# dphoyes/OpenCL-Structure-from-Motion

Hardware: NVIDIA B200
Metric: matched frame-pairs/sec at 1241x376 (higher is better)
Workload: dtype u8

## Files before the change

opencl-structure-from-motion_b200/csrc/outliers.cu:

```cuda
#include "visocu_internal.cuh"
#include "outliers.cuh"
#include <cstdio>
#include <cstdlib>
#include <cstring>
#include <mutex>
#include <type_traits>
#include <utility>
#include <vector>

namespace {

constexpr int NIL = 0xFFFF;
constexpr uint16_t DEAD = 0xFFFF;

__host__ __device__ inline int ro_edge_capacity(int n) { return (int)(3.04f * (float)n) + 64; }
__host__ __device__ inline size_t ro_smem_bytes(int n) {
  return (((size_t)12 * ro_edge_capacity(n) + 15) & ~(size_t)15) + (size_t)4 * n + 16;
}

struct Mesh {
  uint16_t* __restrict__ nx; uint16_t* __restrict__ pv; uint16_t* __restrict__ og;
  const uint32_t* __restrict__ pt;
  int* bump; int ecap; volatile int* fail;
  int guard;

  __device__ __forceinline__ int org(int e) const { return og[e]; }
  __device__ __forceinline__ int dest(int e) const { return og[e ^ 1]; }
  __device__ __forceinline__ int onext(int e) const { return nx[e]; }
  __device__ __forceinline__ int oprev(int e) const { return pv[e]; }
  __device__ __forceinline__ int lnext(int e) const { return pv[e ^ 1]; }
  __device__ __forceinline__ int rprev(int e) const { return nx[e ^ 1]; }
  __device__ __forceinline__ int px(int v) const { return (int)(pt[v] & 0xFFFFu); }
  __device__ __forceinline__ int py(int v) const { return (int)(pt[v] >> 16); }
  __device__ __forceinline__ bool tick() { return --guard >= 0; }
  __device__ __forceinline__ int ccw(int a, int b, int c) const { return ccw_pts(pt[a], pt[b], pt[c]); }
  __device__ __forceinline__ long long incircle(int a, int b, int c, int d) const { return incircle_pts(pt[a], pt[b], pt[c], pt[d]); }
  static __device__ __forceinline__ int ccw_pts(uint32_t A, uint32_t B, uint32_t C) {
    const int cx = (int)(C & 0xFFFF), cy = (int)(C >> 16);
    const int ax = (int)(A & 0xFFFF) - cx, ay = (int)(A >> 16) - cy;
    const int bx = (int)(B & 0xFFFF) - cx, by = (int)(B >> 16) - cy;
    return ax * by - ay * bx;
  }
  static __device__ __forceinline__ long long incircle_pts(uint32_t A, uint32_t B, uint32_t C, uint32_t D) {
    const int dx = (int)(D & 0xFFFF), dy = (int)(D >> 16);
    const int adx = (int)(A & 0xFFFF) - dx, ady = (int)(A >> 16) - dy;
    const int bdx = (int)(B & 0xFFFF) - dx, bdy = (int)(B >> 16) - dy;
    const int cdx = (int)(C & 0xFFFF) - dx, cdy = (int)(C >> 16) - dy;
    const int al = adx * adx + ady * ady, bl = bdx * bdx + bdy * bdy, cl = cdx * cdx + cdy * cdy;
    return (long long)al * (bdx * cdy - cdx * bdy) + (long long)bl * (cdx * ady - adx * cdy) + (long long)cl * (adx * bdy - bdx * ady);
  }
};

struct FreeList { int head, tail; };

template <bool W>
__device__ __forceinline__ int make_edge(Mesh& m, FreeList& fl, int a, int b) {
  int e;
  if (fl.head != NIL) {
    e = fl.head;
    fl.head = (e == fl.tail) ? NIL : m.nx[e];
  } else {
    int k = 0;
    if (!W || (threadIdx.x & 31) == 0) k = atomicAdd(m.bump, 1);
    if (W) k = __shfl_sync(0xFFFFFFFFu, k, 0);
    if (k >= m.ecap) { *m.fail = 1; e = 0; } else e = 2 * k;
  }
  m.nx[e] = (uint16_t)e; m.pv[e] = (uint16_t)e; m.og[e] = (uint16_t)a;
  m.nx[e + 1] = (uint16_t)(e + 1); m.pv[e + 1] = (uint16_t)(e + 1); m.og[e + 1] = (uint16_t)b;
  return e;
}
__device__ __forceinline__ void insert_after(Mesh& m, int x, int e) {
  const int n = m.nx[x];
  m.nx[e] = (uint16_t)n; m.pv[e] = (uint16_t)x;
  m.pv[n] = (uint16_t)e; m.nx[x] = (uint16_t)e;
}
__device__ __forceinline__ void unlink(Mesh& m, int e) {
  const int n = m.nx[e], p = m.pv[e];
  m.nx[p] = (uint16_t)n; m.pv[n] = (uint16_t)p;
}
template <bool W>
__device__ __forceinline__ int connect(Mesh& m, FreeList& fl, int a, int b) {
  const int e = make_edge<W>(m, fl, m.dest(a), m.org(b));
  insert_after(m, m.lnext(a), e);
  insert_after(m, b, e ^ 1);
  return e;
}
__device__ __forceinline__ void remove_edge(Mesh& m, FreeList& fl, int e) {
  unlink(m, e); unlink(m, e ^ 1);
  e &= ~1;
  m.og[e] = DEAD; m.og[e + 1] = DEAD;
  if (fl.head == NIL) { fl.head = fl.tail = e; } else { m.nx[e] = (uint16_t)fl.head; fl.head = e; }
}

struct Handles { int ldo, rdo; };

template <bool W>
__device__ Handles merge(Mesh& m, FreeList& fl, Handles L, Handles R, int axis) {
  int ldo = L.ldo, ldi = L.rdo, rdi = R.ldo, rdo = R.rdo;
  if (axis == 1) {
    while (m.py(m.dest(ldo)) < m.py(m.org(ldo)) && m.tick()) ldo = m.rprev(ldo);
    while (m.py(m.dest(m.onext(ldi))) > m.py(m.org(ldi)) && m.tick()) ldi = m.onext(ldi) ^ 1;
    while (m.py(m.dest(rdi)) < m.py(m.org(rdi)) && m.tick()) rdi = m.rprev(rdi);
    while (m.py(m.dest(m.onext(rdo))) > m.py(m.org(rdo)) && m.tick()) rdo = m.onext(rdo) ^ 1;
  }
  bool changed;
  do {
    changed = false;
    if (m.ccw(m.org(ldi), m.dest(ldi), m.org(rdi)) > 0) { ldi = m.lnext(ldi); changed = true; }
    if (m.ccw(m.dest(rdi), m.org(rdi), m.org(ldi)) > 0) { rdi = m.rprev(rdi); changed = true; }
  } while (changed && m.tick());
  int basel = connect<W>(m, fl, rdi ^ 1, ldi);
  if (m.org(ldi) == m.org(ldo)) ldo = basel ^ 1;
  if (m.org(rdi) == m.org(rdo)) rdo = basel;
  while (m.tick()) {
    const int lowerright = m.org(basel), lowerleft = m.dest(basel);
    int lcand = m.onext(basel ^ 1), rcand = m.oprev(basel);
    int upperleft = m.dest(lcand), upperright = m.dest(rcand);
    const int lnx0 = m.onext(lcand), rnx0 = m.oprev(rcand);
    const int lapex0 = m.dest(lnx0), rapex0 = m.dest(rnx0);
    bool leftfinished, rightfinished, ldel0, rdel0, right_first = false;
    if (W) {
      const int lane = threadIdx.x & 31;
      int myv = rapex0;
      myv = lane == 4 ? lapex0 : myv; myv = lane == 3 ? upperright : myv; myv = lane == 2 ? upperleft : myv;
      myv = lane == 1 ? lowerright : myv; myv = lane == 0 ? lowerleft : myv;
      const uint32_t myp = m.pt[myv];
      const int sh = 4 * min(lane, 7);
#define RO_PICK(table) __shfl_sync(0xFFFFFFFFu, myp, (int)(((table) >> sh) & 7u))
      const uint32_t P = RO_PICK(0x01032u), Q = RO_PICK(0x05200u), R = RO_PICK(0x03411u);
      const uint32_t A = RO_PICK(0x20000u), B = RO_PICK(0x01100u), C = RO_PICK(0x13200u), D = RO_PICK(0x35400u);
#undef RO_PICK
      const unsigned cpos = __ballot_sync(0xFFFFFFFFu, Mesh::ccw_pts(P, Q, R) > 0);
      const unsigned ipos = __ballot_sync(0xFFFFFFFFu, Mesh::incircle_pts(A, B, C, D) > 0);
      leftfinished = !(cpos & 1u); rightfinished = !(cpos & 2u);
      ldel0 = !leftfinished && lnx0 != (basel ^ 1) && (cpos & 4u) && (ipos & 4u);
      rdel0 = !rightfinished && rnx0 != basel && (cpos & 8u) && (ipos & 8u);
      right_first = (ipos & 16u) != 0;
    } else {
      leftfinished = m.ccw(upperleft, lowerleft, lowerright) <= 0;
      rightfinished = m.ccw(upperright, lowerleft, lowerright) <= 0;
      ldel0 = !leftfinished && lnx0 != (basel ^ 1) && m.ccw(lowerleft, upperleft, lapex0) > 0 &&
              m.incircle(lowerleft, lowerright, upperleft, lapex0) > 0;
      rdel0 = !rightfinished && rnx0 != basel && m.ccw(lowerright, rapex0, upperright) > 0 &&
              m.incircle(lowerleft, lowerright, upperright, rapex0) > 0;
    }
    if (leftfinished && rightfinished) break;
    if (ldel0) {
      remove_edge(m, fl, lcand);
      lcand = lnx0; upperleft = lapex0;
      while (m.tick()) {
        const int nx = m.onext(lcand);
        if (nx == (basel ^ 1)) break;
        const int apex = m.dest(nx);
        if (m.ccw(lowerleft, upperleft, apex) <= 0) break;
        if (m.incircle(lowerleft, lowerright, upperleft, apex) <= 0) break;
        remove_edge(m, fl, lcand);
        lcand = nx; upperleft = apex;
      }
    }
    if (rdel0) {
      remove_edge(m, fl, rcand);
      rcand = rnx0; upperright = rapex0;
      while (m.tick()) {
        const int nx = m.oprev(rcand);
        if (nx == basel) break;
        const int apex = m.dest(nx);
        if (m.ccw(lowerright, apex, upperright) <= 0) break;
        if (m.incircle(lowerleft, lowerright, upperright, apex) <= 0) break;
        remove_edge(m, fl, rcand);
        rcand = nx; upperright = apex;
      }
    }
    bool right = leftfinished;
    if (!leftfinished && !rightfinished)
      right = (W && !ldel0 && !rdel0) ? right_first : m.incircle(upperleft, lowerleft, lowerright, upperright) > 0;
    if (right) basel = connect<W>(m, fl, rcand, basel ^ 1);
    else basel = connect<W>(m, fl, basel ^ 1, lcand ^ 1);
    if (W) __syncwarp();
  }
  if (axis == 1) {
    while (m.px(m.dest(m.oprev(ldo))) < m.px(m.org(ldo)) && m.tick()) ldo = m.oprev(ldo) ^ 1;
    while (m.px(m.dest(rdo)) > m.px(m.org(rdo)) && m.tick()) rdo = m.lnext(rdo);
  }
  return Handles{ldo, rdo};
}

template <bool W>
__device__ Handles leaf(Mesh& m, FreeList& fl, int v, int n) {
  if (n == 2) {
    const int a = make_edge<W>(m, fl, v, v + 1);
    return Handles{a, a ^ 1};
  }
  const int a = make_edge<W>(m, fl, v, v + 1);
  const int b = make_edge<W>(m, fl, v + 1, v + 2);
  insert_after(m, b, a ^ 1);
  const int area = m.ccw(v, v + 1, v + 2);
  if (area == 0) return Handles{a, b ^ 1};
  const int c = connect<W>(m, fl, b, a);
  if (area > 0) return Handles{a, b ^ 1};
  return Handles{c ^ 1, c};
}

template <int RO_THREADS>
__device__ __forceinline__ int block_scan(int v, int* s_warp, int& total) {
  const int lane = threadIdx.x & 31, wid = threadIdx.x >> 5;
  int incl = v;
#pragma unroll
  for (int o = 1; o < 32; o <<= 1) { const int t = __shfl_up_sync(0xFFFFFFFFu, incl, o); if (lane >= o) incl += t; }
  __syncthreads();
  if (lane == 31) s_warp[wid] = incl;
  __syncthreads();
  int base = 0, tot = 0;
#pragma unroll
  for (int w = 0; w < RO_THREADS / 32; w++) { const int s = s_warp[w]; if (w < wid) base += s; tot += s; }
  total = tot;
  return base + incl - v;
}

__device__ __forceinline__ bool edge_agrees(const visocu_pmatch& a, const visocu_pmatch& b, int method, float flow_tol, float disp_tol) {
  if (method == 0)
    return __fadd_rn(fabsf(__fsub_rn(__fsub_rn(a.u1c, a.u1p), __fsub_rn(b.u1c, b.u1p))),
                     fabsf(__fsub_rn(__fsub_rn(a.v1c, a.v1p), __fsub_rn(b.v1c, b.v1p)))) < flow_tol;
  if (method == 1) return fabsf(__fsub_rn(__fsub_rn(a.u1c, a.u2c), __fsub_rn(b.u1c, b.u2c))) < disp_tol;
  return fabsf(__fsub_rn(__fsub_rn(a.u1p, a.u2p), __fsub_rn(b.u1p, b.u2p))) < disp_tol &&
         __fadd_rn(fabsf(__fsub_rn(__fsub_rn(a.u1c, a.u1p), __fsub_rn(b.u1c, b.u1p))),
                   fabsf(__fsub_rn(__fsub_rn(a.v1c, a.v1p), __fsub_rn(b.v1c, b.v1p)))) < flow_tol;
}

template <int RO_THREADS>
__device__ __forceinline__ void copy_records(visocu_pmatch* dst, const visocu_pmatch* src, const int32_t* list, int n) {
  const int32_t* s = (const int32_t*)src;
  int32_t* d = (int32_t*)dst;
  for (int idx = threadIdx.x; idx < 12 * n; idx += RO_THREADS) {
    const int i = idx / 12, w = idx - 12 * i;
    d[idx] = s[12 * (size_t)list[i] + w];
  }
}

template <int RO_THREADS>
__global__ void __launch_bounds__(RO_THREADS, 1024 / RO_THREADS)
k_remove_outliers(const RoJob* __restrict__ jobs, int method, float flow_tol, float disp_tol, int smem_bytes, int warp_merges) {
  extern __shared__ __align__(16) uint8_t smem[];
  __shared__ int s_warp[RO_THREADS / 32];
  __shared__ int s_bump, s_fail, s_flag, s_more;
  const RoJob J = jobs[blockIdx.x];
  const int tid = threadIdx.x;
  auto now = []() { unsigned long long t; asm volatile("mov.u64 %0, %%globaltimer;" : "=l"(t)); return t; };
  const unsigned long long t_start = now();
  const int n_in = *J.n_in;
  int32_t* src = J.idx;

  const bool pts_mode = J.pts_in != nullptr;
  const int axis0 = J.axis0;
  int n = 0;
  if (pts_mode) {
    n = n_in;
  } else {
    const int per = (n_in + RO_THREADS - 1) / RO_THREADS;
    const int i0 = min(tid * per, n_in), i1 = min(i0 + per, n_in);
    int cnt = 0;
    for (int i = i0; i < i1; i++) cnt += (!J.keep_in || J.keep_in[i]) ? 1 : 0;
    int total;
    int off = block_scan<RO_THREADS>(cnt, s_warp, total);
    n = total;
    for (int i = i0; i < i1; i++) if (!J.keep_in || J.keep_in[i]) src[off++] = i;
  }
  if (tid == 0) { s_bump = 0; s_fail = 0; s_flag = 0; }
  __syncthreads();

  const int ecap = ro_edge_capacity(n);
  const size_t need = ro_smem_bytes(n);
  const int nl = n;
  if (n <= 3 || n > 0x7FF0 || need > (size_t)smem_bytes) {
    if (!pts_mode) copy_records<RO_THREADS>(J.out, J.in, src, n);
    if (tid == 0) { J.result[0] = n; J.result[1] = (n <= 3 && !pts_mode) ? 0 : 1; J.result[2] = 0; J.result[3] = n; }
    return;
  }

  uint16_t* he_nx = (uint16_t*)smem;
  uint16_t* he_pv = he_nx + 2 * ecap;
  uint16_t* he_og = he_pv + 2 * ecap;
  uint32_t* pts = (uint32_t*)(smem + (((size_t)12 * ecap + 15) & ~(size_t)15));
  uint16_t* h_l = J.hnd;
  uint16_t* h_r = h_l + (n / 2 + 2);
  uint16_t* f_h = h_r + (n / 2 + 2);
  uint16_t* f_t = f_h + (n / 2 + 2);
  int npad = 1;
  while (npad < n) npad <<= 1;
  unsigned long long* keys = (unsigned long long*)smem;
  uint16_t* ax = (uint16_t*)(keys + npad);
  uint16_t* ay = ax + n;
  uint16_t* ain = ay + n;
  uint16_t* la = ain + n;
  uint16_t* lb = la + n;
  uint16_t* lc = lb + n;
  uint16_t* nlo = lc + n;
  uint16_t* nsz = nlo + n;
  uint16_t* pre = nsz + n;
  uint8_t* side = (uint8_t*)(pre + n + 1);

  auto bitonic = [&](int m) {
    for (int k = 2; k <= npad; k <<= 1)
      for (int j = k >> 1; j > 0; j >>= 1) {
        for (int t = tid; t < (npad >> 1); t += RO_THREADS) {
          const int i = ((t & ~(j - 1)) << 1) | (t & (j - 1));
          const int p = (j == (k >> 1)) ? (i ^ (k - 1)) : (i | j);
          if (p < m) {
            const unsigned long long a = keys[i], b = keys[p];
            if (a > b) { keys[i] = b; keys[p] = a; }
          }
        }
        __syncthreads();
      }
  };

  if (tid == 0) s_more = 0;
  for (int i = tid; i < npad; i += RO_THREADS) {
    unsigned long long key = ~0ull;
    if (i < nl && (pts_mode || !J.rep || J.rep[src[i]])) {
      int x, y;
      if (pts_mode) { const uint32_t p = J.pts_in[i]; x = (int)(p & 0xFFFFu); y = (int)(p >> 16); }
      else { const visocu_pmatch& r = J.in[src[i]]; x = (int)r.u1c; y = (int)r.v1c; }
      if (x < 0 || y < 0 || x > 8191 || y > 8191) s_fail = 1;
      key = ((unsigned long long)(unsigned)x << 40) | ((unsigned long long)(unsigned)y << 16) | (unsigned)i;
    }
    keys[i] = key;
  }
  __syncthreads();
  bitonic(nl);
  for (int i = tid; i < npad; i += RO_THREADS)
    if (keys[i] != ~0ull && (i + 1 == npad || keys[i + 1] == ~0ull)) s_more = i + 1;
  __syncthreads();
  for (int i = tid; i < s_more; i += RO_THREADS) {
    const unsigned long long key = keys[i];
    if (i > 0 && (keys[i - 1] >> 16) == (key >> 16)) s_flag = 1;
    ax[i] = (uint16_t)(key >> 40); ay[i] = (uint16_t)(key >> 16);
    ain[i] = (uint16_t)key;
  }
  __syncthreads();
  if (s_fail) {
    if (!pts_mode) copy_records<RO_THREADS>(J.out, J.in, src, nl);
    if (tid == 0) { J.result[0] = nl; J.result[1] = 1; J.result[2] = 0; J.result[3] = nl; }
    return;
  }
  if (s_flag) {
    if (!pts_mode) copy_records<RO_THREADS>(J.out, J.in, src, nl);
    if (tid == 0) { J.result[0] = nl; J.result[1] = 2; J.result[2] = 0; J.result[3] = nl; }
    return;
  }
  n = s_more;
  if (n <= 3) {
    if (!pts_mode) copy_records<RO_THREADS>(J.out, J.in, src, nl);
    if (tid == 0) { J.result[0] = nl; J.result[1] = 3; J.result[2] = 0; J.result[3] = nl; }
    return;
  }
  for (int i = tid; i < npad; i += RO_THREADS)
    keys[i] = i < n ? ((unsigned long long)ay[i] << 40) | ((unsigned long long)ax[i] << 16) | (unsigned)i : ~0ull;
  __syncthreads();
  bitonic(n);
  const unsigned long long t_sorted = now();
  uint16_t* xl = la; uint16_t* yl = lb; uint16_t* spare = lc;
  for (int i = tid; i < n; i += RO_THREADS) { xl[i] = (uint16_t)i; yl[i] = (uint16_t)keys[i]; nlo[i] = 0; nsz[i] = (uint16_t)n; }
  __syncthreads();

  int depth = 0;
  {
    const int per = (n + RO_THREADS - 1) / RO_THREADS;
    const int i0 = min(tid * per, n), i1 = min(i0 + per, n);
    for (;; depth++) {
      const int axis = (depth + axis0) & 1;
      uint16_t* from = axis == 0 ? xl : yl;
      uint16_t* other = axis == 0 ? yl : xl;
      if (tid == 0) s_more = 0;
      for (int i = i0; i < i1; i++) {
        const int sz = nsz[i];
        if (sz > 3) side[from[i]] = (uint8_t)((i - nlo[i]) >= (sz >> 1));
      }
      __syncthreads();
      int cnt = 0;
      for (int i = i0; i < i1; i++) cnt += (nsz[i] > 3) ? side[other[i]] : 0;
      int total;
      int run = block_scan<RO_THREADS>(cnt, s_warp, total);
      for (int i = i0; i < i1; i++) { pre[i] = (uint16_t)run; run += (nsz[i] > 3) ? side[other[i]] : 0; }
      if (i1 == n && i0 < n) pre[n] = (uint16_t)run;
      __syncthreads();
      bool more = false;
      for (int i = i0; i < i1; i++) {
        const int sz = nsz[i], lo = nlo[i];
        const int id = other[i];
        if (sz > 3) {
          const int div = sz >> 1;
          const int ones = pre[i] - pre[lo];
          const int s = side[id];
          spare[s ? lo + div + ones : lo + (i - lo - ones)] = (uint16_t)id;
        } else {
          spare[i] = (uint16_t)id;
        }
      }
      __syncthreads();
      for (int i = i0; i < i1; i++) {
        const int sz = nsz[i], lo = nlo[i];
        if (sz > 3) {
          const int div = sz >> 1;
          if (i - lo < div) { nsz[i] = (uint16_t)div; } else { nlo[i] = (uint16_t)(lo + div); nsz[i] = (uint16_t)(sz - div); }
          if (nsz[i] > 3) more = true;
        }
      }
      if (more) s_more = 1;
      if (axis == 0) { uint16_t* t = yl; yl = spare; spare = t; } else { uint16_t* t = xl; xl = spare; spare = t; }
      __syncthreads();
      if (!s_more) break;
      __syncthreads();
    }
  }
  const int maxdepth = depth + 1;
  for (int i = tid; i < n; i += RO_THREADS) {
    const int id = xl[i];
    pts[i] = (uint32_t)ax[id] | ((uint32_t)ay[id] << 16);
    J.vert[i] = ain[id];
  }
  for (int i = tid; i < n / 2 + 2; i += RO_THREADS) { f_h[i] = NIL; f_t[i] = NIL; }
  __syncthreads();

  const unsigned long long t_part = now();
  Mesh m;
  m.nx = he_nx; m.pv = he_pv; m.og = he_og; m.pt = pts; m.bump = &s_bump; m.ecap = ecap; m.fail = &s_fail;
  m.guard = 64 * ecap;
  unsigned long long t_level = now();
  for (int d = maxdepth; d >= 0; d--) {
    auto subtree = [&](int j, auto warp_wide) {
      constexpr bool W = decltype(warp_wide)::value;
      int lo = 0, sz = n;
      for (int t = d - 1; t >= 0; t--) {
        if (sz <= 3) return;
        const int div = sz >> 1;
        if ((j >> t) & 1) { lo += div; sz -= div; } else { sz = div; }
      }
      FreeList fl{NIL, NIL};
      Handles h;
      if (sz <= 3) {
        h = leaf<W>(m, fl, lo, sz);
      } else {
        const int div = sz >> 1;
        const int sl = lo >> 1, sr = (lo + div) >> 1;
        fl.head = f_h[sl]; fl.tail = f_t[sl];
        if (f_h[sr] != NIL) {
          if (fl.head == NIL) { fl.head = f_h[sr]; fl.tail = f_t[sr]; }
          else { m.nx[fl.tail] = f_h[sr]; fl.tail = f_t[sr]; }
        }
        h = merge<W>(m, fl, Handles{h_l[sl], h_r[sl]}, Handles{h_l[sr], h_r[sr]}, (d + axis0) & 1);
      }
      if (m.guard < 0) s_fail = 1;
      if (!W || (tid & 31) == 0) {
        h_l[lo >> 1] = (uint16_t)h.ldo; h_r[lo >> 1] = (uint16_t)h.rdo;
        f_h[lo >> 1] = (uint16_t)fl.head; f_t[lo >> 1] = (uint16_t)fl.tail;
      }
    };
    if (warp_merges && (1 << d) <= RO_THREADS / 32) {
      if ((tid >> 5) < (1 << d)) {
        m.guard = __reduce_min_sync(0xFFFFFFFFu, m.guard);
        subtree(tid >> 5, std::true_type());
      }
    } else {
      for (int j = (tid & 31) * (RO_THREADS / 32) + (tid >> 5); j < (1 << d); j += RO_THREADS) subtree(j, std::false_type());
    }
    __syncthreads();
    if (tid == 0 && d < 7) { const unsigned long long t = now(); J.result[9 + d] = (int32_t)(t - t_level); t_level = t; }
    else if (tid == 0) t_level = now();
    if (s_fail) break;
  }
  if (s_fail) {
    if (!pts_mode) copy_records<RO_THREADS>(J.out, J.in, src, nl);
    if (tid == 0) { J.result[0] = nl; J.result[1] = 3; J.result[2] = s_bump; J.result[3] = nl; }
    return;
  }

  if (J.mesh_out) {
    const int nh = 2 * min(s_bump, ecap), hb = J.he_base, vb = J.v_base;
    for (int e = tid; e < 2 * ecap; e += RO_THREADS) {
      int4 rec = make_int4(hb + e, hb + e, -1, 0);
      if (e < nh) {
        const int o = he_og[e];
        if (o != DEAD) rec = make_int4(hb + he_nx[e], hb + he_pv[e], vb + o, (int)pts[o]);
      }
      J.mesh_out[e] = rec;
    }
    if (tid == 0) {
      J.result[0] = n; J.result[1] = 0; J.result[2] = s_bump; J.result[3] = nl; J.result[4] = hb + h_l[0]; J.result[5] = hb + h_r[0];
    }
    return;
  }

  const unsigned long long t_built = now();
  if (tid == 0) {
    const int start = h_r[0];
    int e = start, guard = 4 * ecap;
    do { he_og[e] |= 0x8000; e = m.lnext(e); } while (e != start && --guard > 0);
    if (guard <= 0) s_fail = 1;
  }
  __syncthreads();
  if (s_fail) {
    if (!pts_mode) copy_records<RO_THREADS>(J.out, J.in, src, nl);
    if (tid == 0) { J.result[0] = nl; J.result[1] = 3; J.result[2] = s_bump; J.result[3] = nl; }
    return;
  }
  unsigned int* support = (unsigned int*)he_nx;
  float* q_d = (float*)he_nx + nl;
  float* q_u = (float*)he_pv;
  float* q_v = q_u + nl;
  uint16_t* vpos = (uint16_t*)(q_v + nl);
  const bool vote_in_smem = (size_t)8 * nl <= (size_t)4 * ecap && (size_t)8 * nl + (size_t)2 * n <= (size_t)4 * ecap;
  for (int i = tid; i < nl; i += RO_THREADS) {
    support[i] = 0;
    if (vote_in_smem) {
      const visocu_pmatch& r = J.in[src[i]];
      q_u[i] = __fsub_rn(r.u1c, r.u1p); q_v[i] = __fsub_rn(r.v1c, r.v1p);
      q_d[i] = method == 1 ? __fsub_rn(r.u1c, r.u2c) : __fsub_rn(r.u1p, r.u2p);
    }
  }
  if (vote_in_smem)
    for (int i = tid; i < n; i += RO_THREADS) vpos[i] = (uint16_t)J.vert[i];
  __syncthreads();
  const int nedge = min(s_bump, ecap);
  for (int k = tid; k < nedge; k += RO_THREADS) {
    const int o0 = he_og[2 * k], o1 = he_og[2 * k + 1];
    if (o0 == DEAD || o1 == DEAD) continue;
    const int t = ((o0 & 0x8000) ? 0 : 1) + ((o1 & 0x8000) ? 0 : 1);
    if (t == 0) continue;
    int pa, pb;
    bool agree;
    if (vote_in_smem) {
      pa = vpos[o0 & 0x7FFF]; pb = vpos[o1 & 0x7FFF];
      const bool flow_ok = __fadd_rn(fabsf(__fsub_rn(q_u[pa], q_u[pb])), fabsf(__fsub_rn(q_v[pa], q_v[pb]))) < flow_tol;
      const bool disp_ok = fabsf(__fsub_rn(q_d[pa], q_d[pb])) < disp_tol;
      agree = method == 0 ? flow_ok : (method == 1 ? disp_ok : (disp_ok && flow_ok));
    } else {
      pa = J.vert[o0 & 0x7FFF]; pb = J.vert[o1 & 0x7FFF];
      agree = edge_agrees(J.in[src[pa]], J.in[src[pb]], method, flow_tol, disp_tol);
    }
    if (agree) {
      atomicAdd(&support[pa], (unsigned)t);
      atomicAdd(&support[pb], (unsigned)t);
    }
  }
  __syncthreads();
  {
    const int per = (nl + RO_THREADS - 1) / RO_THREADS;
    const int i0 = min(tid * per, nl), i1 = min(i0 + per, nl);
    int cnt = 0;
    for (int i = i0; i < i1; i++) cnt += support[i] >= 4u ? 1 : 0;
    int total;
    int off = block_scan<RO_THREADS>(cnt, s_warp, total);
    int32_t* kept = J.vert;
    __syncthreads();
    for (int i = i0; i < i1; i++) if (support[i] >= 4u) kept[off++] = src[i];
    __syncthreads();
    copy_records<RO_THREADS>(J.out, J.in, kept, total);
    if (tid == 0) {
      J.result[0] = total; J.result[1] = 0; J.result[2] = s_bump; J.result[3] = nl;
      const unsigned long long t_end = now();
      J.result[4] = (int32_t)(t_sorted - t_start); J.result[5] = (int32_t)(t_part - t_sorted);
      J.result[6] = (int32_t)(t_built - t_part); J.result[7] = (int32_t)(t_end - t_built);
    }
  }
}

__global__ void k_outlier_keys(const RoJob* __restrict__ jobs, uint32_t* keys, int stride) {
  const RoJob J = jobs[blockIdx.y];
  const int n = *J.n_in;
  uint32_t* out = keys + (size_t)blockIdx.y * stride;
  for (int i = blockIdx.x * blockDim.x + threadIdx.x; i < n; i += gridDim.x * blockDim.x) {
    uint32_t k = 0xFFFFFFFFu;
    if (!J.keep_in || J.keep_in[i]) {
      const int x = (int)J.in[i].u1c, y = (int)J.in[i].v1c;
      if (x >= 0 && y >= 0 && x <= 0xFFFF && y <= 0xFFFF) k = ((uint32_t)x << 16) | (uint32_t)y;
    }
    out[i] = k;
  }
}

}

int visocu_launch_remove_outliers(visocu_ctx* ctx, const RoJob* jobs_dev, int n_jobs, int method, int max_records, cudaStream_t stream) {
  size_t smem = ro_smem_bytes(max_records);
  const size_t smem_max = 227 * 1024 - 256;
  if (smem > smem_max) smem = smem_max;
  if (smem < 16 * 1024) smem = 16 * 1024;
  {
    static std::mutex mtx;
    static bool done[64] = {false};
    std::lock_guard<std::mutex> lock(mtx);
    if (!done[ctx->device & 63]) {
      CU_TRY(ctx, cudaFuncSetAttribute(k_remove_outliers<1024>, cudaFuncAttributeMaxDynamicSharedMemorySize, (int)smem_max));
      CU_TRY(ctx, cudaFuncSetAttribute(k_remove_outliers<512>, cudaFuncAttributeMaxDynamicSharedMemorySize, (int)smem_max));
      CU_TRY(ctx, cudaFuncSetAttribute(k_remove_outliers<256>, cudaFuncAttributeMaxDynamicSharedMemorySize, (int)smem_max));
      done[ctx->device & 63] = true;
    }
  }
  static const int forced = [] { const char* e = getenv("VISOCU_RO_THREADS"); return e ? atoi(e) : 0; }();
  const int threads = forced ? forced : (n_jobs <= 2 ? 1024 : 512);
  static const int warp = [] { const char* e = getenv("VISOCU_RO_WARP"); return (e && e[0] == '0') ? 0 : 1; }();
  const float ft = (float)ctx->param.outlier_flow_tolerance, dt = (float)ctx->param.outlier_disp_tolerance;
  if (threads >= 1024) k_remove_outliers<1024><<<n_jobs, 1024, smem, stream>>>(jobs_dev, method, ft, dt, (int)smem, warp);
  else if (threads >= 512) k_remove_outliers<512><<<n_jobs, 512, smem, stream>>>(jobs_dev, method, ft, dt, (int)smem, warp);
  else k_remove_outliers<256><<<n_jobs, 256, smem, stream>>>(jobs_dev, method, ft, dt, (int)smem, warp);
  CU_LAUNCH_CHECK(ctx);
  return VISOCU_OK;
}

extern "C" int visocu_remove_outliers(visocu_ctx* ctx, int32_t n_jobs, int32_t method, visocu_pmatch* const* inout, const int32_t* n,
                                      int32_t* n_out, int32_t* status) {
  if (!ctx) return VISOCU_EINVAL;
  if (!ctx->configured) return visocu_set_error(ctx, VISOCU_ESTATE, "context not configured");
  if (n_jobs <= 0 || !inout || !n || !n_out || !status) return visocu_set_error(ctx, VISOCU_EINVAL, "bad outlier removal arguments");
  if (method < 0 || method > 2) return visocu_set_error(ctx, VISOCU_EINVAL, "method %d not supported", method);
  CU_TRY(ctx, cudaSetDevice(ctx->device));
  std::vector<RoJob> hj(n_jobs);
  std::vector<size_t> o_in(n_jobs), o_out(n_jobs), o_idx(n_jobs), o_vert(n_jobs), o_res(n_jobs), o_hnd(n_jobs), o_rep(n_jobs);
  std::vector<std::vector<uint8_t> > reps(n_jobs);
  size_t off = align_up(sizeof(RoJob) * n_jobs, 256);
  int maxn = 0;
  for (int j = 0; j < n_jobs; j++) {
    if (n[j] < 0) return visocu_set_error(ctx, VISOCU_EINVAL, "job %d has a negative count", j);
    const size_t cnt = (size_t)n[j] + 1;
    if (n[j] > maxn) maxn = n[j];
    o_in[j] = off; off += align_up(cnt * 48, 256);
    o_out[j] = off; off += align_up(cnt * 48, 256);
    o_idx[j] = off; off += align_up(cnt * 4, 256);
    o_vert[j] = off; off += align_up(cnt * 4, 256);
    o_hnd[j] = off; off += align_up((cnt / 2 + 2) * 8, 256);
    o_rep[j] = off; off += align_up(cnt, 256);
    o_res[j] = off; off += 256;
  }
  int rc = visocu_ensure_scratch(ctx, off);
  if (rc) return rc;
  if ((rc = visocu_ensure_pinned(ctx, align_up(sizeof(RoJob) * n_jobs, 256) + (size_t)n_jobs * 64))) return rc;
  uint8_t* sb = (uint8_t*)ctx->scratch;
  uint8_t* pin = (uint8_t*)ctx->pinned;
  for (int j = 0; j < n_jobs; j++) {
    RoJob& J = hj[j];
    J.in = (const visocu_pmatch*)(sb + o_in[j]); J.keep_in = nullptr; J.out = (visocu_pmatch*)(sb + o_out[j]);
    J.result = (int32_t*)(sb + o_res[j]); J.n_in = J.result + 8;
    J.idx = (int32_t*)(sb + o_idx[j]); J.vert = (int32_t*)(sb + o_vert[j]); J.hnd = (uint16_t*)(sb + o_hnd[j]);
    if (n[j] > 0) CU_COPY(ctx, sb + o_in[j], inout[j], (size_t)n[j] * 48, cudaMemcpyHostToDevice);
    J.rep = nullptr;
    if (n[j] > 3) {
      std::vector<uint32_t> keys((size_t)n[j]);
      for (int i = 0; i < n[j]; i++) {
        const int x = (int)inout[j][i].u1c, y = (int)inout[j][i].v1c;
        keys[i] = (x >= 0 && y >= 0 && x <= 0xFFFF && y <= 0xFFFF) ? ((uint32_t)x << 16) | (uint32_t)y : 0xFFFFFFFFu;
      }
      reps[j].resize((size_t)n[j]);
      if (ro_resolve_duplicates(keys.data(), n[j], reps[j].data())) {
        CU_COPY(ctx, sb + o_rep[j], reps[j].data(), (size_t)n[j], cudaMemcpyHostToDevice);
        J.rep = sb + o_rep[j];
      }
    }
    CU_COPY(ctx, (void*)J.n_in, &n[j], 4, cudaMemcpyHostToDevice);
  }
  memcpy(pin, hj.data(), sizeof(RoJob) * n_jobs);
  CU_COPY(ctx, sb, pin, sizeof(RoJob) * n_jobs, cudaMemcpyHostToDevice);
  if ((rc = visocu_launch_remove_outliers(ctx, (const RoJob*)sb, n_jobs, method, maxn, ctx->stream))) return rc;
  int32_t* pin_res = (int32_t*)(pin + align_up(sizeof(RoJob) * n_jobs, 256));
  for (int j = 0; j < n_jobs; j++) CU_COPY(ctx, pin_res + 16 * j, hj[j].result, 64, cudaMemcpyDeviceToHost);
  CU_TRY(ctx, visocu_stream_wait(ctx));
  for (int j = 0; j < n_jobs; j++) {
    n_out[j] = pin_res[16 * j]; status[j] = pin_res[16 * j + 1];
    if (getenv("VISOCU_RO_STATS") && j == 0)
      fprintf(stderr, "[outliers] n=%d kept=%d status=%d edges=%d (%.2f n) ns: sort %d partition %d build %d vote %d\n", n[j], pin_res[0], pin_res[1],
              pin_res[2], n[j] ? (double)pin_res[2] / n[j] : 0.0, pin_res[4], pin_res[5], pin_res[6], pin_res[7]),
      fprintf(stderr, "[outliers] merge levels 0..6 (ns): %d %d %d %d %d %d %d\n", pin_res[9], pin_res[10], pin_res[11], pin_res[12], pin_res[13], pin_res[14], pin_res[15]);
    if (status[j] == 0 && n_out[j] > 0) CU_COPY(ctx, inout[j], hj[j].out, (size_t)n_out[j] * 48, cudaMemcpyDeviceToHost);
  }
  CU_TRY(ctx, visocu_stream_wait(ctx));
  return VISOCU_OK;
}

extern "C" int32_t visocu_delaunay_edge_capacity(int32_t n_vertices) { return n_vertices > 0 ? ro_edge_capacity(n_vertices) : 0; }

extern "C" int visocu_delaunay_subtrees(visocu_ctx* ctx, const uint32_t* pts, int32_t n_pts, int32_t n_jobs, const int32_t* first,
                                        const int32_t* count, const int32_t* axis, int32_t extra_halfedges, int32_t** mesh,
                                        int32_t* mesh_first, int32_t* n_halfedges, const int32_t** vert, const int32_t** result) {
  if (!ctx) return VISOCU_EINVAL;
  if (!ctx->configured) return visocu_set_error(ctx, VISOCU_ESTATE, "context not configured");
  if (!pts || n_pts <= 0 || n_jobs <= 0 || !first || !count || !axis || extra_halfedges < 0 || !mesh || !mesh_first || !n_halfedges || !vert || !result)
    return visocu_set_error(ctx, VISOCU_EINVAL, "bad subtree arguments");
  CU_TRY(ctx, cudaSetDevice(ctx->device));
  size_t n_he = 0;
  int maxn = 0;
  for (int j = 0; j < n_jobs; j++) {
    if (first[j] < 0 || count[j] < 4 || count[j] > 0x7FF0 || (int64_t)first[j] + count[j] > n_pts)
      return visocu_set_error(ctx, VISOCU_EINVAL, "subtree %d: range [%d, +%d) not inside %d points or size out of range", j, first[j], count[j], n_pts);
    mesh_first[j] = (int32_t)n_he;
    n_he += 2 * (size_t)ro_edge_capacity(count[j]);
    if (count[j] > maxn) maxn = count[j];
  }
  if (n_he + (size_t)extra_halfedges > 0x7FFFFFF0u) return visocu_set_error(ctx, VISOCU_EINVAL, "too many half-edges");
  const size_t d_jobs = 0, d_pts = align_up(sizeof(RoJob) * n_jobs, 256), d_vert = d_pts + align_up((size_t)4 * n_pts, 256);
  const size_t d_res = d_vert + align_up((size_t)4 * n_pts, 256), d_hnd = d_res + (size_t)64 * n_jobs;
  const size_t d_mesh = d_hnd + align_up((size_t)8 * ((size_t)n_pts / 2 + 2 * (size_t)n_jobs), 256), d_end = d_mesh + 16 * n_he;
  const size_t h_res = align_up(sizeof(RoJob) * n_jobs, 256), h_vert = h_res + (size_t)64 * n_jobs, h_mesh = h_vert + align_up((size_t)4 * n_pts, 256);
  const size_t h_end = h_mesh + 16 * (n_he + (size_t)extra_halfedges);
  int rc = visocu_ensure_scratch(ctx, d_end);
  if (rc) return rc;
  if ((rc = visocu_ensure_pinned(ctx, h_end))) return rc;
  uint8_t* sb = (uint8_t*)ctx->scratch;
  uint8_t* pin = (uint8_t*)ctx->pinned;
  RoJob* hj = (RoJob*)pin;
  int32_t* hres = (int32_t*)(pin + h_res);
  size_t hnd_off = 0;
  for (int j = 0; j < n_jobs; j++) {
    RoJob J;
    memset(&J, 0, sizeof J);
    J.result = (int32_t*)(sb + d_res) + 16 * j; J.n_in = J.result + 8;
    J.vert = (int32_t*)(sb + d_vert) + first[j];
    J.hnd = (uint16_t*)(sb + d_hnd) + hnd_off; hnd_off += 4 * ((size_t)count[j] / 2 + 2);
    J.pts_in = (const uint32_t*)(sb + d_pts) + first[j];
    J.mesh_out = (int4*)(sb + d_mesh) + mesh_first[j];
    J.axis0 = axis[j] & 1; J.he_base = mesh_first[j]; J.v_base = first[j];
    hj[j] = J;
    memset(hres + 16 * j, 0, 64);
    hres[16 * j + 1] = -1; hres[16 * j + 8] = count[j];
  }
  CU_COPY(ctx, sb + d_jobs, pin, sizeof(RoJob) * n_jobs, cudaMemcpyHostToDevice);
  CU_COPY(ctx, sb + d_res, hres, (size_t)64 * n_jobs, cudaMemcpyHostToDevice);
  CU_COPY(ctx, sb + d_pts, pts, (size_t)4 * n_pts, cudaMemcpyHostToDevice);
  if ((rc = visocu_launch_remove_outliers(ctx, (const RoJob*)(sb + d_jobs), n_jobs, 0, maxn, ctx->stream))) return rc;
  CU_COPY(ctx, hres, sb + d_res, (size_t)64 * n_jobs, cudaMemcpyDeviceToHost);
  CU_COPY(ctx, pin + h_vert, sb + d_vert, (size_t)4 * n_pts, cudaMemcpyDeviceToHost);
  CU_COPY(ctx, pin + h_mesh, sb + d_mesh, 16 * n_he, cudaMemcpyDeviceToHost);
  CU_TRY(ctx, visocu_stream_wait(ctx));
  ctx->ro_node_calls++;
  for (int j = 0; j < n_jobs; j++) if (hres[16 * j + 1] == 0) ctx->ro_nodes++;
  *mesh = (int32_t*)(pin + h_mesh); *n_halfedges = (int32_t)n_he; *vert = (const int32_t*)(pin + h_vert); *result = hres;
  return VISOCU_OK;
}

int visocu_launch_outlier_keys(visocu_ctx* ctx, const RoJob* jobs_dev, int n_jobs, uint32_t* keys_dev, int stride) {
  int gx = (stride + 255) / 256; if (gx > 64) gx = 64;
  k_outlier_keys<<<dim3(gx, n_jobs), 256, 0, ctx->stream>>>(jobs_dev, keys_dev, stride);
  CU_LAUNCH_CHECK(ctx);
  return VISOCU_OK;
}

bool ro_resolve_duplicates(const uint32_t* keys, int n_records, uint8_t* rep) {
  static thread_local std::vector<uint32_t> kk, seen_words;
  static thread_local std::vector<int32_t> rec;
  kk.clear(); rec.clear();
  for (int i = 0; i < n_records; i++)
    if (keys[i] != 0xFFFFFFFFu) { kk.push_back(keys[i]); rec.push_back(i); }
  const int n = (int)kk.size();
  size_t cap = 64;
  while (cap < (size_t)4 * n) cap <<= 1;
  seen_words.assign(cap, 0xFFFFFFFFu);
  bool dup = false;
  for (int i = 0; i < n && !dup; i++) {
    const uint32_t k = kk[i];
    size_t h = ((size_t)k * 2654435761u) & (cap - 1);
    while (seen_words[h] != 0xFFFFFFFFu) {
      if (seen_words[h] == k) { dup = true; break; }
      h = (h + 1) & (cap - 1);
    }
    seen_words[h] = k;
  }
  if (!dup) return false;
  static thread_local std::vector<unsigned long long> el;
  el.resize((size_t)n + 1);
  for (int i = 0; i < n; i++) el[i] = ((unsigned long long)kk[i] << 32) | (unsigned)i;
  el[n] = ~0ull;
  unsigned seed = 1;
  static thread_local std::vector<std::pair<int, int> > stack;
  stack.clear();
  stack.push_back(std::make_pair(0, n));
  while (!stack.empty()) {
    const int lo = stack.back().first, len = stack.back().second;
    stack.pop_back();
    if (len < 2) continue;
    unsigned long long* v = el.data() + lo;
    if (len == 2) {
      if ((v[0] >> 32) > (v[1] >> 32)) std::swap(v[0], v[1]);
      continue;
    }
    seed = (seed * 1366u + 150889u) % 714025u;
    const unsigned long long pkey = v[seed / (714025u / (unsigned)len + 1u)] >> 32;
    int left = -1, right = len;
    while (left < right) {
      do { left++; } while (left <= right && (v[left] >> 32) < pkey);
      do { right--; } while (left <= right && (v[right] >> 32) > pkey);
      if (left < right) std::swap(v[left], v[right]);
    }
    if (right < len - 2) stack.push_back(std::make_pair(lo + right + 1, len - right - 1));
    if (left > 1) stack.push_back(std::make_pair(lo, left));
  }
  for (int i = 0; i < n_records; i++) rep[i] = 0;
  for (int i = 0; i < n; i++)
    if (i == 0 || (el[i] >> 32) != (el[i - 1] >> 32)) rep[rec[(size_t)(el[i] & 0xFFFFFFFFu)]] = 1;
  return true;
}
```

Before: 58860.

## Use counting sort for point ordering and warp-level k-d partition at deep levels

Replaces the two bitonic sorts of point keys with a bounded counting sort over the x/y coordinate range, using per-bin insertion sort for ties, whenever no bin exceeds a threshold. It also splits the k-d partitioning so that shallow levels run block-wide and deeper subtrees below a node size are handled independently by single warps with ballot-based scans instead of block barriers. The aim is to cut the log^2 barrier-bound sort cost and the per-level __syncthreads overhead in the outlier removal kernel. Counting sort is only enabled by default for small job counts (<=2), with a bitonic fallback. The change also adds a profiling script.

```diff
diff --git a/opencl-structure-from-motion_b200/csrc/outliers.cu b/opencl-structure-from-motion_b200/csrc/outliers.cu
--- a/opencl-structure-from-motion_b200/csrc/outliers.cu
+++ b/opencl-structure-from-motion_b200/csrc/outliers.cu
@@ -239,10 +239,12 @@
 
 template <int RO_THREADS>
 __global__ void __launch_bounds__(RO_THREADS, 1024 / RO_THREADS)
-k_remove_outliers(const RoJob* __restrict__ jobs, int method, float flow_tol, float disp_tol, int smem_bytes, int warp_merges) {
+k_remove_outliers(const RoJob* __restrict__ jobs, int method, float flow_tol, float disp_tol, int smem_bytes, int warp_merges,
+                  int bin_max, int part_node) {
   extern __shared__ __align__(16) uint8_t smem[];
   __shared__ int s_warp[RO_THREADS / 32];
-  __shared__ int s_bump, s_fail, s_flag, s_more;
+  __shared__ int s_bump, s_fail, s_flag, s_more, s_over;
+  __shared__ int s_rng[4];
   const RoJob J = jobs[blockIdx.x];
   const int tid = threadIdx.x;
   auto now = []() { unsigned long long t; asm volatile("mov.u64 %0, %%globaltimer;" : "=l"(t)); return t; };
@@ -314,106 +316,214 @@
       }
   };
 
-  if (tid == 0) s_more = 0;
-  for (int i = tid; i < npad; i += RO_THREADS) {
-    unsigned long long key = ~0ull;
-    if (i < nl && (pts_mode || !J.rep || J.rep[src[i]])) {
-      int x, y;
-      if (pts_mode) { const uint32_t p = J.pts_in[i]; x = (int)(p & 0xFFFFu); y = (int)(p >> 16); }
-      else { const visocu_pmatch& r = J.in[src[i]]; x = (int)r.u1c; y = (int)r.v1c; }
-      if (x < 0 || y < 0 || x > 8191 || y > 8191) s_fail = 1;
-      key = ((unsigned long long)(unsigned)x << 40) | ((unsigned long long)(unsigned)y << 16) | (unsigned)i;
-    }
-    keys[i] = key;
-  }
-  __syncthreads();
-  bitonic(nl);
-  for (int i = tid; i < npad; i += RO_THREADS)
-    if (keys[i] != ~0ull && (i + 1 == npad || keys[i + 1] == ~0ull)) s_more = i + 1;
-  __syncthreads();
-  for (int i = tid; i < s_more; i += RO_THREADS) {
-    const unsigned long long key = keys[i];
-    if (i > 0 && (keys[i - 1] >> 16) == (key >> 16)) s_flag = 1;
-    ax[i] = (uint16_t)(key >> 40); ay[i] = (uint16_t)(key >> 16);
-    ain[i] = (uint16_t)key;
-  }
-  __syncthreads();
+  int* bins = (int*)keys;
+  auto counting = [&](int m, int nb, auto bin, auto place, auto order) -> bool {
+    for (int b = tid; b < nb; b += RO_THREADS) bins[b] = 0;
+    if (tid == 0) s_over = 0;
+    __syncthreads();
+    for (int i = tid; i < m; i += RO_THREADS) { const int b = bin(i); if (b >= 0) atomicAdd(&bins[b], 1); }
+    __syncthreads();
+    const int per = (nb + RO_THREADS - 1) / RO_THREADS;
+    const int b0 = min(tid * per, nb), b1 = min(b0 + per, nb);
+    int cnt = 0, big = 0;
+    for (int b = b0; b < b1; b++) { const int c = bins[b]; cnt += c; big = max(big, c); }
+    if (big > bin_max) s_over = 1;
+    int total;
+    int run = block_scan<RO_THREADS>(cnt, s_warp, total);
+    if (s_over) return false;
+    for (int b = b0; b < b1; b++) { const int c = bins[b]; bins[b] = run; run += c; }
+    __syncthreads();
+    for (int i = tid; i < m; i += RO_THREADS) { const int b = bin(i); if (b >= 0) place(i, atomicAdd(&bins[b], 1)); }
+    __syncthreads();
+    for (int b = tid; b < nb; b += RO_THREADS) order(b, b > 0 ? bins[b - 1] : 0, bins[b]);
+    __syncthreads();
+    return true;
+  };
+
+  uint16_t* in_x = la;
+  uint16_t* in_y = lb;
+  {
+    int x0 = 0x7FFFFFFF, x1 = -1, y0 = 0x7FFFFFFF, y1 = -1, cnt = 0;
+    if (tid == 0) { s_more = 0; s_rng[0] = s_rng[2] = 0x7FFFFFFF; s_rng[1] = s_rng[3] = -1; }
+    __syncthreads();
+    for (int i = tid; i < nl; i += RO_THREADS) {
+      int x = 0xFFFF, y = 0xFFFF;
+      if (pts_mode || !J.rep || J.rep[src[i]]) {
+        if (pts_mode) { const uint32_t p = J.pts_in[i]; x = (int)(p & 0xFFFFu); y = (int)(p >> 16); }
+        else { const visocu_pmatch& r = J.in[src[i]]; x = (int)r.u1c; y = (int)r.v1c; }
+        if (x < 0 || y < 0 || x > 8191 || y > 8191) s_fail = 1;
+        x0 = min(x0, x); x1 = max(x1, x); y0 = min(y0, y); y1 = max(y1, y); cnt++;
+      }
+      in_x[i] = (uint16_t)x; in_y[i] = (uint16_t)y;
+    }
+    x0 = __reduce_min_sync(0xFFFFFFFFu, x0); x1 = __reduce_max_sync(0xFFFFFFFFu, x1);
+    y0 = __reduce_min_sync(0xFFFFFFFFu, y0); y1 = __reduce_max_sync(0xFFFFFFFFu, y1);
+    cnt = __reduce_add_sync(0xFFFFFFFFu, cnt);
+    if ((tid & 31) == 0) {
+      atomicMin(&s_rng[0], x0); atomicMax(&s_rng[1], x1); atomicMin(&s_rng[2], y0); atomicMax(&s_rng[3], y1);
+      atomicAdd(&s_more, cnt);
+    }
+    __syncthreads();
+  }
   if (s_fail) {
     if (!pts_mode) copy_records<RO_THREADS>(J.out, J.in, src, nl);
     if (tid == 0) { J.result[0] = nl; J.result[1] = 1; J.result[2] = 0; J.result[3] = nl; }
     return;
   }
+  n = s_more;
+  const int xmin = s_rng[0], ymin = s_rng[2];
+  bool counted_x = false, counted_y = false;
+  if (bin_max > 0 && n > 0 && s_rng[1] - xmin < 2 * npad)
+    counted_x = counting(
+        nl, s_rng[1] - xmin + 1, [&](int i) { return in_x[i] == 0xFFFF ? -1 : in_x[i] - xmin; },
+        [&](int i, int pos) { ay[pos] = in_y[i]; ain[pos] = (uint16_t)i; },
+        [&](int b, int lo, int hi) {
+          for (int a = lo + 1; a < hi; a++) {
+            const uint32_t v = ((uint32_t)ay[a] << 16) | ain[a];
+            int c = a - 1;
+            for (; c >= lo && (((uint32_t)ay[c] << 16) | ain[c]) > v; c--) { ay[c + 1] = ay[c]; ain[c + 1] = ain[c]; }
+            ay[c + 1] = (uint16_t)(v >> 16); ain[c + 1] = (uint16_t)v;
+          }
+          for (int a = lo; a < hi; a++) ax[a] = (uint16_t)(xmin + b);
+        });
+  if (!counted_x) {
+    for (int i = tid; i < npad; i += RO_THREADS)
+      keys[i] = i < nl && in_x[i] != 0xFFFF
+                    ? ((unsigned long long)in_x[i] << 40) | ((unsigned long long)in_y[i] << 16) | (unsigned)i : ~0ull;
+    __syncthreads();
+    bitonic(nl);
+    for (int i = tid; i < n; i += RO_THREADS) {
+      const unsigned long long key = keys[i];
+      ax[i] = (uint16_t)(key >> 40); ay[i] = (uint16_t)(key >> 16); ain[i] = (uint16_t)key;
+    }
+    __syncthreads();
+  }
+  for (int i = tid + 1; i < n; i += RO_THREADS)
+    if (ax[i - 1] == ax[i] && ay[i - 1] == ay[i]) s_flag = 1;
+  __syncthreads();
   if (s_flag) {
     if (!pts_mode) copy_records<RO_THREADS>(J.out, J.in, src, nl);
     if (tid == 0) { J.result[0] = nl; J.result[1] = 2; J.result[2] = 0; J.result[3] = nl; }
     return;
   }
-  n = s_more;
   if (n <= 3) {
     if (!pts_mode) copy_records<RO_THREADS>(J.out, J.in, src, nl);
     if (tid == 0) { J.result[0] = nl; J.result[1] = 3; J.result[2] = 0; J.result[3] = nl; }
     return;
   }
-  for (int i = tid; i < npad; i += RO_THREADS)
-    keys[i] = i < n ? ((unsigned long long)ay[i] << 40) | ((unsigned long long)ax[i] << 16) | (unsigned)i : ~0ull;
+  uint16_t* xl = la; uint16_t* yl = lb; uint16_t* spare = lc;
+  if (bin_max > 0 && s_rng[3] - ymin < 2 * npad)
+    counted_y = counting(
+        n, s_rng[3] - ymin + 1, [&](int i) { return ay[i] - ymin; }, [&](int i, int pos) { yl[pos] = (uint16_t)i; },
+        [&](int, int lo, int hi) {
+          for (int a = lo + 1; a < hi; a++) {
+            const uint16_t v = yl[a];
+            int c = a - 1;
+            for (; c >= lo && yl[c] > v; c--) yl[c + 1] = yl[c];
+            yl[c + 1] = v;
+          }
+        });
+  if (!counted_y) {
+    for (int i = tid; i < npad; i += RO_THREADS)
+      keys[i] = i < n ? ((unsigned long long)ay[i] << 40) | ((unsigned long long)ax[i] << 16) | (unsigned)i : ~0ull;
+    __syncthreads();
+    bitonic(n);
+    for (int i = tid; i < n; i += RO_THREADS) yl[i] = (uint16_t)keys[i];
+  }
+  const unsigned long long t_sorted = now();
+  for (int i = tid; i < n; i += RO_THREADS) { xl[i] = (uint16_t)i; nlo[i] = 0; nsz[i] = (uint16_t)n; }
   __syncthreads();
-  bitonic(n);
-  const unsigned long long t_sorted = now();
-  uint16_t* xl = la; uint16_t* yl = lb; uint16_t* spare = lc;
-  for (int i = tid; i < n; i += RO_THREADS) { xl[i] = (uint16_t)i; yl[i] = (uint16_t)keys[i]; nlo[i] = 0; nsz[i] = (uint16_t)n; }
-  __syncthreads();
-
-  int depth = 0;
+
+  int maxdepth = 0;
+  for (int s = n; s > 3; s -= s >> 1) maxdepth++;
+  int block_levels = 0;
+  for (int s = n; s > part_node && block_levels < maxdepth; s -= s >> 1) block_levels++;
+  auto level_side = [&](uint16_t* from, int i) {
+    const int sz = nsz[i];
+    if (sz > 3) side[from[i]] = (uint8_t)((i - nlo[i]) >= (sz >> 1));
+  };
+  auto level_place = [&](uint16_t* other, int i) {
+    const int sz = nsz[i], lo = nlo[i];
+    const int id = other[i];
+    if (sz > 3) {
+      const int div = sz >> 1;
+      const int ones = pre[i] - pre[lo];
+      const int s = side[id];
+      spare[s ? lo + div + ones : lo + (i - lo - ones)] = (uint16_t)id;
+    } else {
+      spare[i] = (uint16_t)id;
+    }
+  };
+  auto level_nodes = [&](int i) {
+    const int sz = nsz[i], lo = nlo[i];
+    if (sz > 3) {
+      const int div = sz >> 1;
+      if (i - lo < div) { nsz[i] = (uint16_t)div; } else { nlo[i] = (uint16_t)(lo + div); nsz[i] = (uint16_t)(sz - div); }
+    }
+  };
+  auto rotate = [&](int axis) {
+    if (axis == 0) { uint16_t* t = yl; yl = spare; spare = t; } else { uint16_t* t = xl; xl = spare; spare = t; }
+  };
   {
     const int per = (n + RO_THREADS - 1) / RO_THREADS;
     const int i0 = min(tid * per, n), i1 = min(i0 + per, n);
-    for (;; depth++) {
+    for (int depth = 0; depth < block_levels; depth++) {
       const int axis = (depth + axis0) & 1;
       uint16_t* from = axis == 0 ? xl : yl;
       uint16_t* other = axis == 0 ? yl : xl;
-      if (tid == 0) s_more = 0;
-      for (int i = i0; i < i1; i++) {
-        const int sz = nsz[i];
-        if (sz > 3) side[from[i]] = (uint8_t)((i - nlo[i]) >= (sz >> 1));
-      }
+      for (int i = i0; i < i1; i++) level_side(from, i);
       __syncthreads();
       int cnt = 0;
       for (int i = i0; i < i1; i++) cnt += (nsz[i] > 3) ? side[other[i]] : 0;
       int total;
       int run = block_scan<RO_THREADS>(cnt, s_warp, total);
       for (int i = i0; i < i1; i++) { pre[i] = (uint16_t)run; run += (nsz[i] > 3) ? side[other[i]] : 0; }
-      if (i1 == n && i0 < n) pre[n] = (uint16_t)run;
       __syncthreads();
-      bool more = false;
-      for (int i = i0; i < i1; i++) {
-        const int sz = nsz[i], lo = nlo[i];
-        const int id = other[i];
-        if (sz > 3) {
-          const int div = sz >> 1;
-          const int ones = pre[i] - pre[lo];
-          const int s = side[id];
-          spare[s ? lo + div + ones : lo + (i - lo - ones)] = (uint16_t)id;
-        } else {
-          spare[i] = (uint16_t)id;
+      for (int i = i0; i < i1; i++) level_place(other, i);
+      __syncthreads();
+      for (int i = i0; i < i1; i++) level_nodes(i);
+      rotate(axis);
+      __syncthreads();
+    }
+  }
+  if (block_levels < maxdepth) {
+    const int lane = tid & 31;
+    const unsigned lt = (1u << lane) - 1u;
+    uint16_t* const xl0 = xl; uint16_t* const yl0 = yl; uint16_t* const spare0 = spare;
+    for (int j = tid >> 5; j < (1 << block_levels); j += RO_THREADS / 32) {
+      int lo = 0, sz = n;
+      for (int t = block_levels - 1; t >= 0; t--) {
+        const int div = sz >> 1;
+        if ((j >> t) & 1) { lo += div; sz -= div; } else { sz = div; }
+      }
+      const int end = lo + sz;
+      xl = xl0; yl = yl0; spare = spare0;
+      for (int depth = block_levels; depth < maxdepth; depth++) {
+        const int axis = (depth + axis0) & 1;
+        uint16_t* from = axis == 0 ? xl : yl;
+        uint16_t* other = axis == 0 ? yl : xl;
+        for (int i = lo + lane; i < end; i += 32) level_side(from, i);
+        __syncwarp();
+        int run = 0;
+        for (int b = lo; b < end; b += 32) {
+          const int i = b + lane;
+          const bool one = i < end && nsz[i] > 3 && side[other[i]];
+          const unsigned bal = __ballot_sync(0xFFFFFFFFu, one);
+          if (i < end) pre[i] = (uint16_t)(run + __popc(bal & lt));
+          run += __popc(bal);
         }
-      }
-      __syncthreads();
-      for (int i = i0; i < i1; i++) {
-        const int sz = nsz[i], lo = nlo[i];
-        if (sz > 3) {
-          const int div = sz >> 1;
-          if (i - lo < div) { nsz[i] = (uint16_t)div; } else { nlo[i] = (uint16_t)(lo + div); nsz[i] = (uint16_t)(sz - div); }
-          if (nsz[i] > 3) more = true;
-        }
-      }
-      if (more) s_more = 1;
-      if (axis == 0) { uint16_t* t = yl; yl = spare; spare = t; } else { uint16_t* t = xl; xl = spare; spare = t; }
-      __syncthreads();
-      if (!s_more) break;
-      __syncthreads();
-    }
-  }
-  const int maxdepth = depth + 1;
+        __syncwarp();
+        for (int i = lo + lane; i < end; i += 32) level_place(other, i);
+        __syncwarp();
+        for (int i = lo + lane; i < end; i += 32) level_nodes(i);
+        rotate(axis);
+        __syncwarp();
+      }
+    }
+    xl = xl0; yl = yl0; spare = spare0;
+    for (int depth = block_levels; depth < maxdepth; depth++) rotate((depth + axis0) & 1);
+    __syncthreads();
+  }
   for (int i = tid; i < n; i += RO_THREADS) {
     const int id = xl[i];
     pts[i] = (uint32_t)ax[id] | ((uint32_t)ay[id] << 16);
@@ -557,7 +667,7 @@
     __syncthreads();
     copy_records<RO_THREADS>(J.out, J.in, kept, total);
     if (tid == 0) {
-      J.result[0] = total; J.result[1] = 0; J.result[2] = s_bump; J.result[3] = nl;
+      J.result[0] = total; J.result[1] = 0; J.result[2] = s_bump; J.result[3] = nl | (counted_x ? 1 << 16 : 0) | (counted_y ? 1 << 17 : 0);
       const unsigned long long t_end = now();
       J.result[4] = (int32_t)(t_sorted - t_start); J.result[5] = (int32_t)(t_part - t_sorted);
       J.result[6] = (int32_t)(t_built - t_part); J.result[7] = (int32_t)(t_end - t_built);
@@ -600,10 +710,13 @@
   static const int forced = [] { const char* e = getenv("VISOCU_RO_THREADS"); return e ? atoi(e) : 0; }();
   const int threads = forced ? forced : (n_jobs <= 2 ? 1024 : 512);
   static const int warp = [] { const char* e = getenv("VISOCU_RO_WARP"); return (e && e[0] == '0') ? 0 : 1; }();
+  static const int bin_env = [] { const char* e = getenv("VISOCU_RO_BIN_MAX"); return e ? atoi(e) : -1; }();
+  const int bin_max = bin_env >= 0 ? bin_env : (n_jobs <= 2 ? 64 : 0);
+  static const int part_node = [] { const char* e = getenv("VISOCU_RO_PART_NODE"); return e && atoi(e) > 3 ? atoi(e) : e ? 3 : 128; }();
   const float ft = (float)ctx->param.outlier_flow_tolerance, dt = (float)ctx->param.outlier_disp_tolerance;
-  if (threads >= 1024) k_remove_outliers<1024><<<n_jobs, 1024, smem, stream>>>(jobs_dev, method, ft, dt, (int)smem, warp);
-  else if (threads >= 512) k_remove_outliers<512><<<n_jobs, 512, smem, stream>>>(jobs_dev, method, ft, dt, (int)smem, warp);
-  else k_remove_outliers<256><<<n_jobs, 256, smem, stream>>>(jobs_dev, method, ft, dt, (int)smem, warp);
+  if (threads >= 1024) k_remove_outliers<1024><<<n_jobs, 1024, smem, stream>>>(jobs_dev, method, ft, dt, (int)smem, warp, bin_max, part_node);
+  else if (threads >= 512) k_remove_outliers<512><<<n_jobs, 512, smem, stream>>>(jobs_dev, method, ft, dt, (int)smem, warp, bin_max, part_node);
+  else k_remove_outliers<256><<<n_jobs, 256, smem, stream>>>(jobs_dev, method, ft, dt, (int)smem, warp, bin_max, part_node);
   CU_LAUNCH_CHECK(ctx);
   return VISOCU_OK;
 }
@@ -669,6 +782,8 @@
     if (getenv("VISOCU_RO_STATS") && j == 0)
       fprintf(stderr, "[outliers] n=%d kept=%d status=%d edges=%d (%.2f n) ns: sort %d partition %d build %d vote %d\n", n[j], pin_res[0], pin_res[1],
               pin_res[2], n[j] ? (double)pin_res[2] / n[j] : 0.0, pin_res[4], pin_res[5], pin_res[6], pin_res[7]),
+      fprintf(stderr, "[outliers] sorts: x %s, y %s\n", pin_res[1] == 0 && (pin_res[3] & 0x10000) ? "counting" : "bitonic",
+              pin_res[1] == 0 && (pin_res[3] & 0x20000) ? "counting" : "bitonic"),
       fprintf(stderr, "[outliers] merge levels 0..6 (ns): %d %d %d %d %d %d %d\n", pin_res[9], pin_res[10], pin_res[11], pin_res[12], pin_res[13], pin_res[14], pin_res[15]);
     if (status[j] == 0 && n_out[j] > 0) CU_COPY(ctx, inout[j], hj[j].out, (size_t)n_out[j] * 48, cudaMemcpyDeviceToHost);
   }
diff --git a/profiles/profile_outlier_phases.py b/profiles/profile_outlier_phases.py
--- /dev/null
+++ b/profiles/profile_outlier_phases.py
@@ -0,0 +1,57 @@
+import os
+import re
+import subprocess
+import sys
+
+HERE = os.path.dirname(os.path.dirname(os.path.abspath(__file__)))
+
+CHILD = r'''
+import sys
+sys.path[:0] = [sys.argv[1], sys.argv[1] + '/opencl-structure-from-motion_b200']
+import numpy as np
+import visocu_py as V
+n, reps = int(sys.argv[2]), int(sys.argv[3])
+rng = np.random.default_rng(3)
+def make(n):
+    m = np.zeros(n, V.P_MATCH)
+    cells = rng.choice(620 * 188, size=n, replace=False)
+    m['u1c'] = (cells % 620) * 2 + 6; m['v1c'] = (cells // 620) * 2 + 6
+    flow = rng.integers(-3, 4, (n, 2))
+    m['u1p'] = m['u1c'] - flow[:, 0]; m['v1p'] = m['v1c'] - flow[:, 1]
+    return m
+ctx = V.Context(0)
+ctx.configure(V.Params(), 1241, 376, 4)
+lists = [make(n) for _ in range(64)]
+for _ in range(reps + 2):
+    ctx.remove_outliers(lists, 0)
+ctx.close()
+'''
+
+
+def phases(tree, n, threads, reps):
+    env = dict(os.environ, VISOCU_RO_THREADS=str(threads), VISOCU_RO_STATS='1')
+    r = subprocess.run([sys.executable, '-c', CHILD, tree, str(n), str(reps)], env=env, capture_output=True, text=True)
+    if r.returncode:
+        raise RuntimeError(r.stderr[-2000:])
+    rows = [tuple(int(v) for v in t) for t in
+            re.findall(r'ns: sort (\d+) partition (\d+) build (\d+) vote (\d+)', r.stderr)][2:]
+    sorts = re.findall(r'sorts: x (\w+), y (\w+)', r.stderr)
+    med = [sorted(c)[len(c) // 2] / 1e3 for c in zip(*rows)]
+    return med, (sorts[-1] if sorts else ('-', '-'))
+
+
+def main():
+    tree = os.path.abspath(sys.argv[1]) if len(sys.argv) > 1 else HERE
+    reps = int(sys.argv[2]) if len(sys.argv) > 2 else 15
+    print('tree %s' % tree)
+    print('| points | threads | sort | partition | build | vote | total (us) | x / y order |')
+    print('|---|---|---|---|---|---|---|---|')
+    for n in (900, 4100):
+        for threads in (256, 512, 1024):
+            med, sorts = phases(tree, n, threads, reps)
+            print('| %d | %d | %.0f | %.0f | %.0f | %.0f | %.0f | %s |' % (n, threads, *med, sum(med), ' / '.join(sorts)))
+            sys.stdout.flush()
+
+
+if __name__ == '__main__':
+    main()
```

Measured after the change: 59220, median of 6. No clear change (+0.6%).
